# federicomegler/sq-learn

Measured on AMD Instinct MI355X. Metric: q-means fit samples/sec (Lloyd samples*iterations/s, delta-means + tomography noise), higher is better.
Workload: dtype fp32; 1 GPU; model=q-means k=1024 delta=0.5 (10000000 x 256 synthetic), global_batch=10000000, seq_len=256, parallelism=dp1

## Files before the change

### sq_learn_amd/csrc/estep_f32.hip

```cpp
#include "common.h"
#include "band.h"
#include "f16_tile.h"
#include "sq_api.h"

namespace sq {

constexpr int kMaxCand = 16;

#ifndef SQ_SPLIT_ACC_ALL
#define SQ_SPLIT_ACC_ALL 1
#endif
template <int KSD, int TOP = 2>
__global__ void __launch_bounds__(256, 1) estep_f32_kernel(
    const float* __restrict__ X, const _Float16* __restrict__ C, const float* __restrict__ xn,
    int* __restrict__ labels, float* __restrict__ mind, long long* __restrict__ ovf_rows,
    int* __restrict__ ovf_count, double* __restrict__ part, long long n, int k_pad, float alpha,
    float inv_alpha2, float delta_s, RngKey key, long long row_offset, int ovf_cap,
    const long long* __restrict__ rlist, const int* __restrict__ rcount,
    const float* __restrict__ cmax2_p, long long* __restrict__ mrows, int* __restrict__ mcand,
    int* __restrict__ multi_count, unsigned char* __restrict__ xflag, long long mcap) {
  const float Cm = cmax2_p ? sqrtf(*cmax2_p) * (1.0f + 0x1p-16f) : 0.0f;
  constexpr bool SPLIT_ACC = SQ_SPLIT_ACC_ALL || TOP == 3;
  constexpr float kEps3 =
      SPLIT_ACC ? (3.0f * 0x1p-22f + (KSD * 16 + 18.0f) * 0x1p-24f + 2.0f * KSD * 16 * 0x1p-34f) *
// ... 157 lines not shown

  int G = 0;
  stage(0);
  load_raw(blk);
  sync_tile();
  split();
  double my_inertia = 0.0;

  for (; blk < nblk; blk += gridDim.x) {
    const long long row0 = blk * ROWS + wave * 32;
    if constexpr (!PREFETCH) {
      if (blk != (long long)blockIdx.x) {
        load_raw(blk);
        asm volatile("s_waitcnt vmcnt(0)" ::: "memory");
        split();
      }
    }
#pragma unroll
    for (int i = 0; i < 16; ++i) {
      m1[i] = m2[i] = m3[i] = __builtin_inff();
      i1[i] = i2[i] = 0;
      if constexpr (TOP == 3) {
        m4[i] = __builtin_inff();
        i3[i] = 0;
      }
    }
    f32x16 pA0, pA1, pB0, pB1;
    stage(G + 1);
    tile_step(buf(G), pA0, pA1, true, pA0, pA1, 0, false);
    sync_tile();
    int t = 0;
    while (true) {
      if (t + 1 >= n_tiles) {
        if constexpr (PREFETCH) load_raw(blk + gridDim.x);
        tile_step(smem, pB0, pB1, false, pA0, pA1, t, true);
        break;
      }
      stage(G + 2);
      tile_step(buf(G + 1), pB0, pB1, true, pA0, pA1, t, true);
      sync_tile();
      ++t;
      ++G;
      if (t + 1 >= n_tiles) {
        if constexpr (PREFETCH) load_raw(blk + gridDim.x);
        tile_step(smem, pA0, pA1, false, pB0, pB1, t, true);
        break;
      }
      stage(G + 2);
      tile_step(buf(G + 1), pA0, pA1, true, pB0, pB1, t, true);
      sync_tile();
      ++t;
      ++G;
    }
    ++G;

    float R1[16], R2[16];
    int RI[16];
#pragma unroll
    for (int i = 0; i < 16; ++i) { R1[i] = m1[i]; R2[i] = m2[i]; RI[i] = i1[i]; }
#pragma unroll
    for (int o = 16, c = 8; o >= 2; o >>= 1, c >>= 1) {
      const bool hi = (r32 & o) != 0;
#pragma unroll
      for (int j = 0; j < c; ++j) {
        const float ra = R1[j], rb = R1[c + j], sa = R2[j], sb = R2[c + j];
        const int ia = RI[j], ib = RI[c + j];
        const float s1 = hi ? ra : rb, s2 = hi ? sa : sb;
        const int si = hi ? ia : ib;
        float k1 = hi ? rb : ra, k2 = hi ? sb : sa;
        int ki = hi ? ib : ia;
        merge(k1, k2, ki, __shfl_xor(s1, o, 64), __shfl_xor(s2, o, 64), __shfl_xor(si, o, 64));
        R1[j] = k1;
        R2[j] = k2;
        RI[j] = ki;
      }
    }
    float q1 = R1[0], q2 = R2[0];
    int qi = RI[0];
    merge(q1, q2, qi, __shfl_xor(R1[0], 1, 64), __shfl_xor(R2[0], 1, 64), __shfl_xor(RI[0], 1, 64));

    const int irow = r32 >> 1;
    const int rloc = acc_row(irow, half);
    const long long grow_local = row0 + rloc;
    const bool owner = ((r32 & 1) == 0) && grow_local < n;
    const float thr = q1 + delta_s;
    const long long gmap = owner ? map_row(grow_local) : 0;
    const float xnv = owner ? xn[gmap] : 0.0f;
    const float e2 = cmax2_p ? 2.0f * kEps3 * (2.0f * alpha * sqrtf(xnv) * Cm + Cm * Cm) : 0.0f;
    const bool unc = cmax2_p && fabsf(q2 - thr) <= e2;
    const bool band2 = q2 <= thr && !unc;
    if (owner) {
      const float dist = fmaxf(xnv + q1 * inv_alpha2, 0.0f);
      mind[gmap] = dist;
      if (!band2 && !unc) labels[gmap] = qi;
      my_inertia += (double)dist;
    }
    const unsigned long long slow = __ballot(owner && (band2 || unc));
    if (slow) {
      const float urow = band_u(key, row_offset + gmap);
#pragma unroll
      for (int i = 0; i < 16; ++i) {
        const unsigned long long sel = slow & ((1ull << (2 * i)) | (1ull << (32 + 2 * i)));
        if (!sel) continue;
        const int src = 32 * half + 2 * i;
        const bool mine = (slow >> src) & 1ull;
        const float thr_i = __shfl(thr, src, 64);
        const float u_i = __shfl(urow, src, 64);
        const float e2_i = __shfl(e2, src, 64);
        const bool unc_i = __shfl(unc ? 1 : 0, src, 64) != 0;
        const long long g_i = __shfl(gmap, src, 64);
        const int c1 = (mine && m1[i] <= thr_i) ? 1 : 0;
        const int c2 = (mine && m2[i] <= thr_i) ? 1 : 0;
        int c3 = 0;
        bool v3;
        const float lim = thr_i + e2_i;
        bool nr = fabsf(m1[i] - thr_i) <= e2_i || fabsf(m2[i] - thr_i) <= e2_i ||
                  fabsf(m3[i] - thr_i) <= e2_i;
        int cc = (m1[i] <= lim ? 1 : 0) + (m2[i] <= lim ? 1 : 0);
        bool last_in;
        if constexpr (TOP == 3) {
          c3 = (mine && m3[i] <= thr_i) ? 1 : 0;
          v3 = mine && m4[i] <= thr_i;
          nr = nr || fabsf(m4[i] - thr_i) <= e2_i;
          cc += m3[i] <= lim ? 1 : 0;
          last_in = m4[i] <= lim;
        } else {
          v3 = mine && m3[i] <= thr_i;
          last_in = m3[i] <= lim;
        }
        const bool row_unc =
            cmax2_p && mine &&
            (unc_i || ((__ballot(mine && nr) >> (32 * half)) & 0xFFFFFFFFull) != 0ull);
        const int cl = c1 + c2 + c3;
        int incl = cl, cinc = cc;
#pragma unroll
        for (int o = 1; o < 32; o <<= 1) {
          const int v = __shfl_up(incl, o, 32);
          const int w = __shfl_up(cinc, o, 32);
          if (r32 >= o) {
            incl += v;
            cinc += w;
          }
        }
        const int ctot = __shfl(cinc, 32 * half + 31, 64);
        const bool untr = ((__ballot(mine && last_in) >> (32 * half)) & 0xFFFFFFFFull) != 0ull;
        const bool to_multi = row_unc && mrows && !untr && ctot >= 2 && ctot <= kMaxCand;
        if (to_multi) {
          int* mc = mcand + g_i * (kMaxCand + 1);
          const int b0 = 1 + cinc - cc;
          if (cc > 0) mc[b0] = i1[i];
          if (cc > 1) mc[b0 + 1] = i2[i];
          if constexpr (TOP == 3) {
            if (cc > 2) mc[b0 + 2] = i3[i];
          }
        }
        const int total = __shfl(incl, 32 * half + 31, 64);
        const bool ovf = ((__ballot(v3) >> (32 * half)) & 0xFFFFFFFFull) != 0ull;
        const int r = band_rank(u_i, total > 0 ? total : 1);
        const bool hit = cl > 0 && r >= incl - cl && r < incl;
        int myj;
        if constexpr (TOP == 3) {
          const int x1 = i1[i];
          const int x2 = cl >= 2 ? i2[i] : 0x7fffffff, x3 = cl >= 3 ? i3[i] : 0x7fffffff;
          const int s_lo = min(x1, min(x2, x3)), s_hi = max(x1, max(x2, x3));
          const int s_mid = (int)((unsigned)x1 + (unsigned)x2 + (unsigned)x3 - (unsigned)s_lo -
                                  (unsigned)s_hi);
          const int kk = r - (incl - cl);
          myj = kk == 0 ? s_lo : (kk == 1 ? (cl == 2 ? min(max(x1, x2), s_hi) : s_mid) : s_hi);
        } else {
          const int x1 = i1[i], x2 = i2[i];
          const int lo_j = min(x1, x2), hi_j = max(x1, x2);
          myj = cl == 1 ? x1 : (r - (incl - cl) == 0 ? lo_j : hi_j);
        }
        const unsigned long long hb = __ballot(hit) >> (32 * half);
        const int pl = hb ? __ffsll((long long)hb) - 1 : 0;
        const int jsel = __shfl(myj, 32 * half + pl, 64);
        if (mine && r32 == 2 * i) {
          const long long g = gmap;
          bool to_ovf = ovf;
          if (row_unc) {
            to_ovf = false;
            if (to_multi) {
              const long long slot = atomicAdd(multi_count, 1);
              if (slot < mcap) {
                mrows[slot] = g;
                if (xflag) xflag[slot] = 1;
                mcand[g * (kMaxCand + 1)] = ctot;
                labels[g] = -1;
              } else {
                to_ovf = true;
              }
            } else if (ctot == 1 && !untr) {
              labels[g] = qi;
            } else {
              to_ovf = true;
            }
          }
          if (to_ovf) {
            const int slot = atomicAdd(ovf_count, 1);
            if (slot < ovf_cap) ovf_rows[slot] = g;
            labels[g] = -1;
          } else if (!row_unc) {
            labels[g] = jsel;
          }
        }
      }
    }
    if constexpr (PREFETCH) {
      if (blk + gridDim.x < nblk) split();
    }
  }
  my_inertia = wave_sum(my_inertia);
  if (lane == 0) part[(size_t)blockIdx.x * NW + wave] = my_inertia;
  asm volatile("s_waitcnt vmcnt(0)" ::: "memory");
}

constexpr int kGapCand = 4;
struct __align__(16) GapRec {
  float da, err;
  float g[kGapCand];
  unsigned ids[2];
};

constexpr int kX64Waves = 4;

#ifndef SQ_X64_STAMP
#define SQ_X64_STAMP 0
#endif
#if SQ_X64_STAMP
constexpr int kStampWaves = 8192;
constexpr int kStampN = 12;
__device__ unsigned long long g_x64_stamps[kStampWaves * kStampN];
#define SQ_STAMP_NOW() __builtin_amdgcn_s_memtime()
#endif

template <int KSD>
using X64Ring = TileRing<KSD, kX64Waves>;

template <int KSD>
struct X64RowSets {
  static constexpr int value = KSD <= 16 ? 2 : 1;
};
constexpr int kX64Pfd = 2;

template <int KSD, int RS>
__global__ void __launch_bounds__(kX64Waves * 64) estep_x64_kernel(
    const _Float16* __restrict__ Xh, const float* __restrict__ X, const _Float16* __restrict__ C,
    const float* __restrict__ Cm, const float* __restrict__ xn, const float* __restrict__ cmax2_p,
    int* __restrict__ labels, float* __restrict__ mind, long long* __restrict__ dense_rows,
    int* __restrict__ dense_count, long long* __restrict__ mrows, int* __restrict__ mcand,
    int* __restrict__ multi_count, long long n, int k_pad, float alpha, float delta_s,
    RngKey key, long long row_offset, int dense_cap, int qbits, const long long* __restrict__ rlist,
    const int* __restrict__ rcount, float* __restrict__ ub, float* __restrict__ lb,
    int* __restrict__ mflag) {
  constexpr int NW = kX64Waves;
  constexpr int DX = KSD * 16;
  using Ring = X64Ring<KSD>;
  constexpr int KT = Ring::KT, NS = Ring::NS, SK = Ring::SK, RING = Ring::RING;
  constexpr int ROWS = NW * 32 * RS;
  extern __shared__ __attribute__((aligned(16))) unsigned char smem[];
  auto buf = [&](int g) -> unsigned char* { return Ring::buf(smem, g); };
  int* cand_all = reinterpret_cast<int*>(smem + Ring::BYTES);
  int* cnt_all = cand_all + NW * RS * 32 * kMaxCand;

  const int tid = threadIdx.x;
  const int lane = tid & 63;
  const int wave = __builtin_amdgcn_readfirstlane(tid >> 6);
  const int r32 = lane & 31;
  const int half = lane >> 5;
  const int n_tiles = k_pad / kTileN;
  const long long ne = rlist ? min((long long)*rcount, n) : n;
  auto row_at = [&](long long pos) -> long long {
    const long long q = pos < ne ? pos : ne - 1;
    return rlist ? rlist[q] : q;
  };
  const long long nblk = (ne + ROWS - 1) / ROWS;
  long long blk = blockIdx.x;
  if (blk >= nblk) return;
  const uint32_t qmask = (1u << qbits) - 1u;
  const uint32_t keep = ~qmask;
  const float Ch = 2.0f * sqrtf(*cmax2_p) * (1.0f + 0x1p-16f);
  const float pack_rel = ldexpf(1.0f, qbits - 23) + 0x1p-15f;
  const float sub_rel = 0x1p-21f * sqrtf((float)DX);

  auto stage = [&](int U) { Ring::stage(C, smem, U, n_tiles); };

  f16x8 ah[RS][KSD];
  auto load_a = [&](long long b) {
    sq::load_a(ah, half, [&](int st) {
      return Xh + (size_t)row_at(b * ROWS + (wave * RS + st) * 32 + r32) * DX;
    });
  };
  const f16x8 aug = aug_frag(half);
  const int rl_own = acc_row(r32 >> 1, half);
  float xn_cur[RS], xn_nxt[RS];
  auto load_xn = [&](long long b, float (&dst)[RS]) {
#pragma unroll
    for (int st = 0; st < RS; ++st) dst[st] = xn[row_at(b * ROWS + (wave * RS + st) * 32 + rl_own)];
  };

  float m1[RS][16], m2[RS][16], m3[RS][16];
  const int lane_off = f16op::lane_off(half, r32);
  auto ins = [&](int st, int i, float v, uint32_t q) {
    const float p = and_or(v, keep, q);
    const float a1 = m1[st][i], a2 = m2[st][i];
    m3[st][i] = vmed3(a2, p, m3[st][i]);
    m2[st][i] = vmed3(a1, p, a2);
    m1[st][i] = vmin(a1, p);
  };
  typedef f32x16 Acc[RS][2];
  auto sub_step = [&](auto S_, const unsigned char* cur, Acc& acc, const Acc& o, int t_prev,
                      bool do_epi) {
    constexpr int S = decltype(S_)::value;
    constexpr int K0 = S * SK, K1 = (S + 1) * SK < KT ? (S + 1) * SK : KT;
    const uint32_t q0 = (uint32_t)(t_prev * 2), q1 = q0 + 1u;
    const unsigned char* hb = cur + lane_off;
    f16x8 b0[2], b1[2];
    b0[0] = ldb(hb + f16op::frag_off(0, 0));
    b1[0] = ldb(hb + f16op::frag_off(1, 0));
#pragma unroll
    for (int ks = K0; ks < K1; ++ks) {
      const int c = (ks - K0) & 1, nx = c ^ 1;
      if (ks + 1 < K1) {
        b0[nx] = ldb(hb + f16op::frag_off(0, ks + 1 - K0));
        b1[nx] = ldb(hb + f16op::frag_off(1, ks + 1 - K0));
      }
#pragma unroll
      for (int st = 0; st < RS; ++st) {
        const f16x8 A = ks < KSD ? ah[st][ks] : aug;
        acc[st][0] = __builtin_amdgcn_mfma_f32_32x32x16_f16(A, b0[c], acc[st][0], 0, 0, 0);
        acc[st][1] = __builtin_amdgcn_mfma_f32_32x32x16_f16(A, b1[c], acc[st][1], 0, 0, 0);
      }
      if (do_epi) {
#pragma unroll
        for (int e = (ks * 16 * RS) / KT; e < ((ks + 1) * 16 * RS) / KT; ++e) {
          ins(e / 16, e % 16, o[e / 16][0][e % 16], q0);
          ins(e / 16, e % 16, o[e / 16][1][e % 16], q1);
        }
      }
      __builtin_amdgcn_sched_barrier(0);
    }
  };
  auto epi_all = [&](const Acc& o, int t_prev) {
    const uint32_t q0 = (uint32_t)(t_prev * 2), q1 = q0 + 1u;
#pragma unroll
    for (int st = 0; st < RS; ++st)
#pragma unroll
      for (int i = 0; i < 16; ++i) {
        ins(st, i, o[st][0][i], q0);
        ins(st, i, o[st][1][i], q1);
      }
  };
#if SQ_X64_STAMP
  unsigned long long st_sync = 0, st_sync0 = 0, st_post = 0, st_sweep = 0, st_blocks = 0;
  unsigned long long st_stage = 0, st_cand = 0, st_aload = 0, st_rmin = 0, st_cl = 0, st_ub = 0;
  const unsigned long long st_t0 = SQ_STAMP_NOW();
  bool st_first = true;
#endif
  auto sync_tile = [&]() {
#if SQ_X64_STAMP
    const unsigned long long sa = SQ_STAMP_NOW();
#endif
    Ring::sync();
#if SQ_X64_STAMP
    const unsigned long long sw = SQ_STAMP_NOW() - sa;
    st_sync += sw;
    if (st_first) st_sync0 += sw;
    st_first = false;
#endif
  };

  int U = 0;
  auto tile = [&](Acc& acc, const Acc& o, int t_prev, bool do_epi) {
#pragma unroll
    for (int st = 0; st < RS; ++st) acc[st][0] = acc[st][1] = (f32x16){0};
    static_for<NS>([&](auto S_) {
      stage(U + RING - 1);
      sub_step(S_, buf(U), acc, o, t_prev, do_epi);
      sync_tile();
      ++U;
    });
  };

  stage(0);
  stage(1);
  load_a(blk);
  load_xn(blk, xn_cur);
  asm volatile("s_waitcnt vmcnt(0)" ::: "memory");
  __builtin_amdgcn_s_barrier();

  for (; blk < nblk; blk += gridDim.x) {
#pragma unroll
    for (int st = 0; st < RS; ++st)
#pragma unroll
      for (int i = 0; i < 16; ++i) m1[st][i] = m2[st][i] = m3[st][i] = __builtin_inff();
    if constexpr (RS == 1) {
      Acc pA, pB;
      tile(pA, pA, 0, false);
      int t = 0;
      while (true) {
        if (t + 1 >= n_tiles) {
          load_a(blk + gridDim.x);
          load_xn(blk + gridDim.x, xn_nxt);
          epi_all(pA, t);
          break;
        }
        tile(pB, pA, t, true);
        ++t;
        if (t + 1 >= n_tiles) {
          load_a(blk + gridDim.x);
          load_xn(blk + gridDim.x, xn_nxt);
          epi_all(pB, t);
          break;
        }
        tile(pA, pB, t, true);
        ++t;
      }
    } else {
      f32x16 cA[RS], cB[RS];
      constexpr int PFD = kX64Pfd;
      f16x8 bq[PFD + 1];
      static_assert(NS == 1, "row sets need whole tiles per LDS slot");
#if SQ_X64_STAMP
      const unsigned long long sw0 = SQ_STAMP_NOW();
      st_first = true;
      ++st_blocks;
#endif
      for (int t = 0; t < n_tiles; ++t) {
#if SQ_X64_STAMP
        const unsigned long long sg0 = SQ_STAMP_NOW();
#endif
        stage(U + RING - 1);
#if SQ_X64_STAMP
        st_stage += SQ_STAMP_NOW() - sg0;
#endif
        tile_prime<KT>(buf(U), lane_off, bq);
        half_pass<0>(buf(U), lane_off, ah, aug, bq, cA, cB, (uint32_t)(2 * t - 1), t > 0, ins);
        half_pass<1>(buf(U), lane_off, ah, aug, bq, cB, cA, (uint32_t)(2 * t), true, ins);
        sync_tile();
        ++U;
      }
#if SQ_X64_STAMP
      const unsigned long long sl0 = SQ_STAMP_NOW();
#endif
      load_a(blk + gridDim.x);
      load_xn(blk + gridDim.x, xn_nxt);
#if SQ_X64_STAMP
      st_aload += SQ_STAMP_NOW() - sl0;
#endif
      half_drain(cB, (uint32_t)(2 * n_tiles - 1), ins);
#if SQ_X64_STAMP
      st_sweep += SQ_STAMP_NOW() - sw0;
#endif
    }
#if SQ_X64_STAMP
    const unsigned long long sp0 = SQ_STAMP_NOW();
#endif

#pragma nounroll
    for (int st = 0; st < RS; ++st) {
#if SQ_X64_STAMP
    const unsigned long long sc0 = SQ_STAMP_NOW();
#endif
    const long long row0 = blk * ROWS + (wave * RS + st) * 32;
    int* cand = cand_all + (wave * RS + st) * 32 * kMaxCand;
    int* cnt = cnt_all + (wave * RS + st) * 32;
    float ms1[16], ms2[16], ms3[16];
#pragma unroll
    for (int i = 0; i < 16; ++i) {
      ms1[i] = m1[0][i]; ms2[i] = m2[0][i]; ms3[i] = m3[0][i];
#pragma unroll
      for (int o = 1; o < RS; ++o) {
        const float a1 = m1[o][i], a2 = m2[o][i], a3 = m3[o][i];
        ms1[i] = st == o ? a1 : ms1[i];
        ms2[i] = st == o ? a2 : ms2[i];
        ms3[i] = st == o ? a3 : ms3[i];
      }
    }

    auto row_min = [&](float (&R)[16]) -> float {
#pragma unroll
      for (int o = 16, c = 8; o >= 2; o >>= 1, c >>= 1) {
        const bool hi = (r32 & o) != 0;
#pragma unroll
        for (int j = 0; j < c; ++j) {
          const float lo_v = R[j], hi_v = R[c + j];
          const float keepv = hi ? hi_v : lo_v, sendv = hi ? lo_v : hi_v;
          R[j] = vmin(keepv, __shfl_xor(sendv, o, 64));
        }
      }
      return vmin(R[0], __shfl_xor(R[0], 1, 64));
    };
    float R[16];
#pragma unroll
    for (int i = 0; i < 16; ++i) R[i] = ms1[i];
    const float rmin = row_min(R);
    float xn_own = xn_cur[0];
#pragma unroll
    for (int o = 1; o < RS; ++o) xn_own = st == o ? xn_cur[o] : xn_own;
    const float xsv = alpha * sqrtf(xn_own) * (1.0f + 0x1p-16f);
    const float prod = xsv * Ch;
    const float mag = 0.25f * Ch * Ch + prod;
    const float E = 1.0625f * 0x1p-10f * prod + pack_rel * mag + sub_rel * (xsv + Ch);
    const float T_own = __uint_as_float(__float_as_uint(rmin) & keep) + delta_s + 2.0f * E;

#if SQ_X64_STAMP
    const unsigned long long sc1 = SQ_STAMP_NOW();
    st_rmin += sc1 - sc0;
#endif
    float nc[16];
    float Tr[16];
#pragma unroll
    for (int i = 0; i < 16; ++i) Tr[i] = __shfl(T_own, 32 * half + 2 * i, 64);
    int* const sink = cnt_all + NW * RS * 32 + wave * 64 + lane;
#pragma unroll
    for (int i = 0; i < 16; ++i) {
      const float T = Tr[i];
      nc[i] = ms1[i] > T ? ms1[i] : (ms2[i] > T ? ms2[i] : ms3[i]);
      const int rl = acc_row(i, half);
      auto jof = [&](float p) -> int {
        const uint32_t q = __float_as_uint(p) & qmask;
        return (int)((q >> 1) * kTileN + (q & 1u) * 32u) + r32;
      };
      const unsigned long long b1 = __ballot(ms1[i] <= T), b2 = __ballot(ms2[i] <= T);
      const unsigned long long b3 = __ballot(ms3[i] <= T);
      const uint32_t b1l = (uint32_t)b1, b1h = (uint32_t)(b1 >> 32);
      const uint32_t b2l = (uint32_t)b2, b2h = (uint32_t)(b2 >> 32);
      const int c1 = __popc(half ? b1h : b1l), c2 = __popc(half ? b2h : b2l);
      const bool d3 = (half ? (uint32_t)(b3 >> 32) : (uint32_t)b3) != 0u;
      const int s1 = (int)__builtin_amdgcn_mbcnt_hi(b1h, __builtin_amdgcn_mbcnt_lo(b1l, 0u)) -
                     (half ? __popc(b1l) : 0);
      const int s2 = c1 + (int)__builtin_amdgcn_mbcnt_hi(b2h, __builtin_amdgcn_mbcnt_lo(b2l, 0u)) -
                     (half ? __popc(b2l) : 0);
      *((ms1[i] <= T && s1 < kMaxCand) ? cand + rl * kMaxCand + s1 : sink) = jof(ms1[i]);
      *((ms2[i] <= T && s2 < kMaxCand) ? cand + rl * kMaxCand + s2 : sink) = jof(ms2[i]);
      *(r32 == 0 ? cnt + rl : sink) = c1 + c2 + (d3 ? kMaxCand + 1 : 0);
    }
#if SQ_X64_STAMP
    const unsigned long long sc2 = SQ_STAMP_NOW();
    st_cl += sc2 - sc1;
#endif
    float ub_own = 0.f, lb_own = 0.f;
    if (ub) {
      const float ncmin = row_min(nc);
      const float ia2 = 1.0f / (alpha * alpha);
      const float d1 = (__uint_as_float(__float_as_uint(rmin) & keep) + E) * ia2;
      const float d2 = (__uint_as_float(__float_as_uint(ncmin) & keep) - E) * ia2;
      const float marg = 0x1p-20f * (xn_own + fabsf(d1) + fabsf(d2));
      ub_own = sqrtf(fmaxf(xn_own + d1 + marg, 0.f)) * (1.0f + 0x1p-20f);
      lb_own = sqrtf(fmaxf(xn_own + d2 - marg, 0.f)) * (1.0f - 0x1p-20f);
    }
    asm volatile("s_waitcnt lgkmcnt(0)" ::: "memory");
    __builtin_amdgcn_wave_barrier();
#if SQ_X64_STAMP
    st_cand += SQ_STAMP_NOW() - sc0;
    st_ub += SQ_STAMP_NOW() - sc2;
#endif

    const bool valid = row0 + r32 < ne;
    const long long g = row_at(row0 + r32);
    if (ub) {
      const int src = ((r32 & 3) + 4 * ((r32 >> 3) & 3)) * 2 + 32 * ((r32 >> 2) & 1);
      const float u = __shfl(ub_own, src, 64), l = __shfl(lb_own, src, 64);
      if (valid && half == 0) {
        ub[g] = u;
        lb[g] = cnt[r32] <= kMaxCand ? l : 0.0f;
      }
    }
    const int c_r = cnt[r32];
    const bool dense = c_r > kMaxCand;
    const bool multi = valid && !dense && c_r >= 2;
    if (mflag && valid && half == 0 && !multi) mflag[g] = 0;
    if (valid && half == 0) {
      if (dense) {
        const int s = atomicAdd(dense_count, 1);
        if (s < dense_cap) dense_rows[s] = g;
        labels[g] = -1;
      } else if (c_r == 1) {
        labels[g] = cand[r32 * kMaxCand];
        mind[g] = -1.0f;
      }
    }
    const bool mrow = multi && half == 0;
    const unsigned long long mm = __ballot(mrow);
    const int nm = __popcll(mm);
    int mbase = 0;
    if (lane == 0 && nm) mbase = atomicAdd(multi_count, nm);
    mbase = __shfl(mbase, 0, 64);
    if (mrow) {
      const long long slot = (long long)mbase + __popcll(mm & ((1ull << lane) - 1ull));
      if (mflag) mflag[g] = slot < n ? 1 : 0;
      if (slot < n) {
        mrows[slot] = g;
        int* mc = mcand + g * (kMaxCand + 1);
        mc[0] = c_r;
        for (int c = 0; c < c_r; ++c) mc[1 + c] = cand[r32 * kMaxCand + c];
      } else {
        const int s2 = atomicAdd(dense_count, 1);
        if (s2 < dense_cap) dense_rows[s2] = g;
        labels[g] = -1;
      }
    }
    asm volatile("s_waitcnt lgkmcnt(0)" ::: "memory");
    __builtin_amdgcn_wave_barrier();
    }
#pragma unroll
    for (int st = 0; st < RS; ++st) xn_cur[st] = xn_nxt[st];
#if SQ_X64_STAMP
    st_post += SQ_STAMP_NOW() - sp0;
#endif
  }
  asm volatile("s_waitcnt vmcnt(0)" ::: "memory");
#if SQ_X64_STAMP
  const int sidx = blockIdx.x * NW + wave;
  if (lane == 0 && sidx < kStampWaves) {
    unsigned long long* o = g_x64_stamps + (size_t)sidx * kStampN;
    o[0] = SQ_STAMP_NOW() - st_t0; o[1] = st_sweep; o[2] = st_sync; o[3] = st_sync0;
    o[4] = st_post; o[5] = st_blocks; o[6] = st_stage; o[7] = st_cand; o[8] = st_aload;
    o[9] = st_rmin; o[10] = st_cl; o[11] = st_ub;
  }
#endif
}

constexpr int kBfLdsK = 2048;
template <int PER>
__global__ void __launch_bounds__(256) bounds_filter_kernel(
    const int* __restrict__ labels, float* __restrict__ ub, float* __restrict__ lb,
    const double* __restrict__ shift, const double* __restrict__ smax, long long n, double delta,
    long long* __restrict__ rlist, int* __restrict__ rcount, const int* __restrict__ mflag,
    long long* __restrict__ mrows, int* __restrict__ multi_count, const float* __restrict__ cc,
    const int* __restrict__ fidx, int nf, int k, int rec_on, int it_now, int it_lo,
    long long* __restrict__ mrows_b, int* __restrict__ count_b, float* __restrict__ corr,
    int* __restrict__ rec_count) {
  constexpr int kBoundsChunk = PER * 256;
  __shared__ int wsum[4], wsum_b[4];
  __shared__ int lbase[3];
  __shared__ double sf_s[65];
  __shared__ double sh_s[kBfLdsK];
  __shared__ float cm_s[kBfLdsK];
  const bool tab = k <= kBfLdsK;
  const int tid = threadIdx.x, lane = tid & 63, wv = tid >> 6;
  if (tid < nf) sf_s[tid] = shift[fidx[tid]];
  if (tab)
    for (int j = tid; j < k; j += 256) {
      sh_s[j] = shift[j];
      cm_s[j] = nf > 0 ? cc[(size_t)k * nf + j] : 0.0f;
    }
  __syncthreads();
  if (tid == 0) {
    double m = 0.0;
    for (int f = 0; f < nf; ++f) m = fmax(m, sf_s[f]);
    sf_s[nf] = m;
  }
  __syncthreads();
  const double sm = *smax;
  const long long c0 = (long long)blockIdx.x * kBoundsChunk;
  unsigned long long act = 0, rec = 0, recb = 0;
  constexpr int B = PER % 4 == 0 ? 4 : 1;
  for (int p0 = 0; p0 < PER; p0 += B) {
    int lv[B], mfv[B];
    float ubv[B], lbv[B];
    bool inb[B];
#pragma unroll
    for (int q = 0; q < B; ++q) {
      const long long i = c0 + (long long)(p0 + q) * 256 + tid;
      inb[q] = i < n;
      const long long ii = inb[q] ? i : 0;
      lv[q] = inb[q] ? labels[ii] : -1;
      if (corr && inb[q]) corr[ii] = 0.0f;
      ubv[q] = ub[ii];
      lbv[q] = lb[ii];
      mfv[q] = mflag[ii];
    }
    double shv[B];
    float cmv[B];
#pragma unroll
    for (int q = 0; q < B; ++q) {
      const int l = lv[q];
      if (tab) {
        shv[q] = l >= 0 ? sh_s[l] : 1e300;
        cmv[q] = l >= 0 ? cm_s[l] : 0.0f;
      } else {
        shv[q] = l >= 0 ? shift[l] : 1e300;
        cmv[q] = (l >= 0 && nf > 0) ? cc[(size_t)k * nf + l] : 0.0f;
      }
    }
#pragma unroll
    for (int q = 0; q < B; ++q) {
      if (!inb[q]) continue;
      const int p = p0 + q;
      const long long i = c0 + (long long)p * 256 + tid;
      const int l = lv[q];
      const double u = (double)ubv[q] + shv[q];
      auto wbound = [&](double lb0) -> double {
        double w = lb0 - sm;
        if (l >= 0 && nf > 0 && w > 0.0) {
          const double wc = fmin(w, fmax((double)cmv[q] - u, lb0 - sf_s[nf]));
          if (wc > 0.0 && wc * wc - u * u > delta * (1.0 + 1e-9) + 1e-30) {
            w = wc;
          } else {
            const float* cl = cc + (size_t)l * nf;
            if ((nf & 3) == 0) {
              for (int f = 0; f < nf; f += 4) {
                const float4 c4 = *reinterpret_cast<const float4*>(cl + f);
                w = fmin(w, fmax((double)c4.x - u, lb0 - sf_s[f]));
                w = fmin(w, fmax((double)c4.y - u, lb0 - sf_s[f + 1]));
                w = fmin(w, fmax((double)c4.z - u, lb0 - sf_s[f + 2]));
                w = fmin(w, fmax((double)c4.w - u, lb0 - sf_s[f + 3]));
              }
            } else {
              for (int f = 0; f < nf; ++f) w = fmin(w, fmax((double)cl[f] - u, lb0 - sf_s[f]));
            }
          }
        }
        return w;
      };
      const double w = wbound((double)lbv[q]);
      const bool holds = l >= 0 && w > 0.0 && w * w - u * u > delta * (1.0 + 1e-9) + 1e-30;
      if (!holds) {
        act |= 1ull << p;
      } else {
        ub[i] = (float)u * (1.0f + 0x1p-22f);
        lb[i] = (float)w * (1.0f - 0x1p-22f);
        if (mfv[q]) {
          if (rec_on && mfv[q] >= it_lo + 2 && mfv[q] <= it_now + 1) recb |= 1ull << p;
          else rec |= 1ull << p;
        }
      }
    }
  }
  const int mine = __popcll(act) | (__popcll(rec) << 16);
  const int mine_b = __popcll(recb);
  int incl = mine, incl_b = mine_b;
#pragma unroll
  for (int o = 1; o < 64; o <<= 1) {
    const int v = __shfl_up(incl, o, 64);
    const int vb = __shfl_up(incl_b, o, 64);
    if (lane >= o) {
      incl += v;
      incl_b += vb;
    }
  }
  if (lane == 63) {
    wsum[wv] = incl;
    wsum_b[wv] = incl_b;
  }
  __syncthreads();
  int before = 0, total = 0, before_b = 0, total_b = 0;
#pragma unroll
  for (int w2 = 0; w2 < 4; ++w2) {
    before += w2 < wv ? wsum[w2] : 0;
    total += wsum[w2];
    before_b += w2 < wv ? wsum_b[w2] : 0;
    total_b += wsum_b[w2];
  }
  if (tid < 4) {
    const int add = tid == 0 ? (total & 0xffff) : (tid == 2 ? total_b : (total >> 16));
    int* ctr = tid == 0 ? rcount : (tid == 1 ? multi_count : (tid == 2 ? count_b : rec_count));
    const int at = (add && ctr) ? atomicAdd(ctr, add) : 0;
    if (tid < 3) lbase[tid] = at;
  }
  __syncthreads();
  const int ex = before + incl - mine;
  int pos = lbase[0] + (ex & 0xffff);
  while (act) {
    const int p = __ffsll((long long)act) - 1;
    rlist[pos++] = c0 + (long long)p * 256 + tid;
    act &= act - 1;
  }
  int mpos = lbase[1] + (ex >> 16);
  while (rec) {
    const int p = __ffsll((long long)rec) - 1;
    mrows[mpos++] = c0 + (long long)p * 256 + tid;
    rec &= rec - 1;
  }
  int bpos = lbase[2] + before_b + incl_b - mine_b;
  while (recb) {
    const int p = __ffsll((long long)recb) - 1;
    mrows_b[bpos++] = c0 + (long long)p * 256 + tid;
    recb &= recb - 1;
  }
}

struct MultiRec {
  GapRec* rec = nullptr;
  int* mflag = nullptr;
  int it_now = 0, it_lo = 0;
  int ring = 0;
  const _Float16* dsh = nullptr;
  const float* dq = nullptr;
  long long dsh_stride = 0;
  long long* mrows_b = nullptr;
  int* count_b = nullptr;
  int* n_done = nullptr;
  long long* mrows_mv = nullptr;
  int* count_mv = nullptr;
};
struct Ovf2 {
  void* rows = nullptr;
  int* count = nullptr;
};

extern "C" int sq_bounds_filter(const void* labels, void* ub, void* lb, const void* shift,
                                const void* smax, long long n, double delta, void* rlist,
                                void* rcount, const void* mflag, void* mrows, void* multi_count,
                                const void* cc, const void* fidx, int nf, int k, void* stream,
                                void* corr, void* rec_count, int rec_on, int it_now, int it_lo,
                                void* mrows_b, void* count_b) {
  if (rec_on && (it_now < 1 || it_lo < 1 || it_lo > it_now || !mrows_b || !count_b))
    return (int)hipErrorInvalidValue;
  if (n <= 0) return 0;
  if (!mflag || !mrows || !multi_count) return (int)hipErrorInvalidValue;
  if (nf < 0 || nf > 64 || (nf > 0 && (!cc || !fidx || k <= nf))) return (int)hipErrorInvalidValue;
  hipStream_t st = (hipStream_t)stream;
  static long long resident = 0;
  if (resident == 0) {
    int dev = 0, cus = 0, per_cu = 0;
    hipGetDevice(&dev);
    hipDeviceGetAttribute(&cus, hipDeviceAttributeMultiprocessorCount, dev);
    hipOccupancyMaxActiveBlocksPerMultiprocessor(&per_cu, (const void*)bounds_filter_kernel<32>,
                                                 256, 0);
    resident = (long long)(cus > 0 ? cus : 256) * (per_cu > 0 ? per_cu : 4);
  }
  auto pick = [&](int per) { return (n + per * 256LL - 1) / (per * 256LL) <= resident; };
  static const int per_env = [] {
    const char* e = getenv("SQ_BF_PER");
    return e ? atoi(e) : 0;
  }();
  int per = pick(8) ? 8 : pick(16) ? 16 : pick(20) ? 20 : pick(32) ? 32 : 64;
  if (per_env == 4 || per_env == 8 || per_env == 16 || per_env == 20 || per_env == 32 ||
      per_env == 64)
    per = per_env;
  const long long blocks = (n + per * 256LL - 1) / (per * 256LL);
  auto kern = per == 4 ? bounds_filter_kernel<4> : per == 8 ? bounds_filter_kernel<8>
            : per == 16 ? bounds_filter_kernel<16> : per == 20 ? bounds_filter_kernel<20>
            : per == 32 ? bounds_filter_kernel<32> : bounds_filter_kernel<64>;
  hipLaunchKernelGGL(kern, dim3((unsigned)blocks),
                     dim3(256), 0, st, (const int*)labels, (float*)ub, (float*)lb,
                     (const double*)shift, (const double*)smax, n, delta, (long long*)rlist,
// ... 1209 lines not shown
```

### sq_learn_amd/csrc/f16_tile.h

```cpp
#pragma once
#include "common.h"
#include <utility>

namespace sq {

typedef _Float16 f16x8 __attribute__((ext_vector_type(8)));
typedef float f32x16 __attribute__((ext_vector_type(16)));

constexpr int kTileN = 64;

SQ_DEV float vmin(float a, float b) {
  float r;
  asm("v_min_f32 %0, %1, %2" : "=v"(r) : "v"(a), "v"(b));
  return r;
}
SQ_DEV float and_or(float a, uint32_t m, uint32_t q) {
  float r;
  asm("v_and_or_b32 %0, %1, %2, %3" : "=v"(r) : "v"(a), "s"(m), "v"(q));
  return r;
}
SQ_DEV float vmed3(float a, float b, float c) {
  float r;
  asm("v_med3_f32 %0, %1, %2, %3" : "=v"(r) : "v"(a), "v"(b), "v"(c));
  return r;
}

template <typename F, int... I>
SQ_DEV void static_for_impl(F&& f, std::integer_sequence<int, I...>) {
  (f(std::integral_constant<int, I>{}), ...);
}
template <int N, typename F>
SQ_DEV void static_for(F&& f) {
  static_for_impl(f, std::make_integer_sequence<int, N>{});
}

__host__ __device__ constexpr int acc_row(int i, int half) {
  return (i & 3) + 8 * (i >> 2) + 4 * half;
}

namespace f16op {
constexpr int kChunkElems = kTileN * 8;
constexpr int kChunkBytes = kChunkElems * 2;
constexpr int kStepBytes = 2 * kChunkBytes;
constexpr int kColHalfBytes = 32 * 16;
constexpr int kNormElems = 3;

__host__ __device__ constexpr int hi_bytes(int ksd) { return (ksd + 1) * kStepBytes; }
__host__ __device__ constexpr int tile_bytes(int ksd) { return (2 * ksd + 1) * kStepBytes; }

__host__ __device__ constexpr size_t row_base(int d_pad, int j) {
  return (size_t)(j >> 6) * (2 * (d_pad / 8) + 2) * kChunkElems + (size_t)(j & 63) * 8;
}
__host__ __device__ constexpr size_t hi_off(int f) { return (size_t)(f >> 3) * kChunkElems + (f & 7); }
__host__ __device__ constexpr size_t lo_off(int d_pad, int f) {
  return (size_t)(d_pad / 8 + 2 + (f >> 3)) * kChunkElems + (f & 7);
}

__host__ __device__ constexpr int lane_off(int half, int r32) { return (half * 64 + r32) * 16; }
__host__ __device__ constexpr int frag_off(int h, int ks) { return h * kColHalfBytes + ks * kStepBytes; }
}

SQ_DEV f16x8 ldb(const unsigned char* p) { return *reinterpret_cast<const f16x8*>(p); }

template <int KSD, int NW>
struct TileRing {
  static constexpr int RING = 3;
  static constexpr int KT = KSD + 1;
  static constexpr int NS = (KT + 23) / 24;
  static constexpr int SK = (KT + NS - 1) / NS;
  static constexpr int SLOT = SK * f16op::kStepBytes;
  static constexpr int PIECES = SLOT / f16op::kChunkBytes;
  static constexpr int PPW = (PIECES + NW - 1) / NW;
  static constexpr int BYTES = RING * SLOT;

  static SQ_DEV unsigned char* buf(unsigned char* smem, int g) { return smem + (g % RING) * SLOT; }

  static SQ_DEV void stage(const _Float16* C, unsigned char* smem, int U, int n_tiles) {
    const int t = (NS == 1 ? U : U / NS) % n_tiles;
    const int sub = NS == 1 ? 0 : U % NS;
    const int npc = 2 * min(SK, KT - sub * SK);
    const unsigned char* tile = reinterpret_cast<const unsigned char*>(C) +
                                (size_t)t * f16op::tile_bytes(KSD) + (size_t)sub * SLOT;
    unsigned char* dst = buf(smem, U);
#pragma unroll
    for (int i = 0; i < PPW; ++i) {
      const int wave = __builtin_amdgcn_readfirstlane((int)threadIdx.x >> 6);
      const int p = wave + NW * i < npc ? wave + NW * i : npc - 1;
      const int lane = threadIdx.x & 63;
      __builtin_amdgcn_global_load_lds(
          (const __attribute__((address_space(1))) void*)(tile + p * f16op::kChunkBytes + lane * 16),
          (__attribute__((address_space(3))) void*)(dst + p * f16op::kChunkBytes), 16, 0, 0);
    }
  }
  static SQ_DEV void sync() {
    asm volatile("s_waitcnt vmcnt(%0)" ::"n"(PPW) : "memory");
    __builtin_amdgcn_s_barrier();
  }
};

static inline int resident_blocks(const void* kern, int threads, size_t lds) {
  int dev = 0, cus = 0, per_cu = 0;
  (void)hipGetDevice(&dev);
  (void)hipDeviceGetAttribute(&cus, hipDeviceAttributeMultiprocessorCount, dev);
  (void)hipOccupancyMaxActiveBlocksPerMultiprocessor(&per_cu, kern, threads, lds);
  return (cus > 0 ? cus : 256) * (per_cu > 0 ? per_cu : 1);
}

SQ_DEV f16x8 a_frag(const _Float16* row, int half, int ks) {
  return *reinterpret_cast<const f16x8*>(row + half * 8 + ks * 16);
}
template <int RS, int KSD, typename Row>
SQ_DEV void load_a(f16x8 (&ah)[RS][KSD], int half, Row&& row) {
#pragma unroll
  for (int st = 0; st < RS; ++st) {
    const _Float16* xr = row(st);
#pragma unroll
    for (int ks = 0; ks < KSD; ++ks) ah[st][ks] = a_frag(xr, half, ks);
  }
}
SQ_DEV f16x8 aug_frag(int half) {
  f16x8 aug = (f16x8)0;
  if (half == 0) { aug[0] = aug[1] = aug[2] = (_Float16)1.0f; }
  return aug;
}

template <int KT, int NB>
SQ_DEV void tile_prime(const unsigned char* cur, int lane_off, f16x8 (&bq)[NB]) {
#pragma unroll
  for (int j = 0; j < NB - 1; ++j) bq[j] = ldb(cur + lane_off + f16op::frag_off(j / KT, j % KT));
}
template <int H, int KSD, int RS, int NB, typename Epi>
SQ_DEV void half_pass(const unsigned char* cur, int lane_off, const f16x8 (&ah)[RS][KSD],
                      const f16x8& aug, f16x8 (&bq)[NB], f32x16 (&acc)[RS],
                      const f32x16 (&o)[RS], uint32_t qo, bool do_epi, Epi&& epi) {
  constexpr int KT = KSD + 1, PFD = NB - 1;
#pragma unroll
  for (int st = 0; st < RS; ++st) acc[st] = (f32x16){0};
#pragma unroll
  for (int ks = 0; ks < KT; ++ks) {
    const int g = H * KT + ks;
    if (g + PFD < 2 * KT)
      bq[(g + PFD) % NB] = ldb(cur + lane_off + f16op::frag_off((g + PFD) / KT, (g + PFD) % KT));
#pragma unroll
    for (int st = 0; st < RS; ++st)
      acc[st] = __builtin_amdgcn_mfma_f32_32x32x16_f16(ks < KSD ? ah[st][ks] : aug, bq[g % NB],
                                                       acc[st], 0, 0, 0);
    if (do_epi) {
#pragma unroll
      for (int e = (ks * 16 * RS) / KT; e < ((ks + 1) * 16 * RS) / KT; ++e)
        epi(e / 16, e % 16, o[e / 16][e % 16], qo);
    }
    __builtin_amdgcn_sched_barrier(0);
  }
}
template <int RS, typename Epi>
SQ_DEV void half_drain(const f32x16 (&o)[RS], uint32_t qo, Epi&& epi) {
#pragma unroll
  for (int st = 0; st < RS; ++st)
#pragma unroll
    for (int i = 0; i < 16; ++i) epi(st, i, o[st][i], qo);
}

SQ_DEV void tile_from_zero(const unsigned char* tile, int lane_off, const _Float16* row, int half,
                           int ksd, f32x16& c0, f32x16& c1) {
  const f16x8 aug = aug_frag(half);
  c0 = (f32x16){0};
  c1 = (f32x16){0};
  for (int ks = 0; ks < ksd + 1; ++ks) {
    const f16x8 av = ks < ksd ? a_frag(row, half, ks) : aug;
    const f16x8 b0 = ldb(tile + lane_off + f16op::frag_off(0, ks));
    const f16x8 b1 = ldb(tile + lane_off + f16op::frag_off(1, ks));
    c0 = __builtin_amdgcn_mfma_f32_32x32x16_f16(av, b0, c0, 0, 0, 0);
    c1 = __builtin_amdgcn_mfma_f32_32x32x16_f16(av, b1, c1, 0, 0, 0);
  }
}

}
```

Measured before the change: 16.86 billion samples*iter/s.

## Interleave centroid tile staging with MFMA passes and trim candidate-list epilogue

Replaces the bulk per-tile staging call with per-piece global-to-LDS loads spread across the MFMA k-steps of each half pass, tracked by explicit ring-slot and look-ahead tile counters. The epilogue insertion into the top-3 lists is also spread per MFMA and hand-written as inline asm for multi-row-set configs. The goal is to hide load issue and VALU work behind matrix instructions. Separately, the candidate-count code skips the second and third ballot processing when no lane has a qualifying second or third candidate. This adds scheduling complexity, and the inline asm and AGPR constraint hints may increase register pressure.

```diff
diff --git a/sq_learn_amd/csrc/estep_f32.hip b/sq_learn_amd/csrc/estep_f32.hip
--- a/sq_learn_amd/csrc/estep_f32.hip
+++ b/sq_learn_amd/csrc/estep_f32.hip
@@ -483,11 +483,21 @@
   float m1[RS][16], m2[RS][16], m3[RS][16];
   const int lane_off = f16op::lane_off(half, r32);
   auto ins = [&](int st, int i, float v, uint32_t q) {
-    const float p = and_or(v, keep, q);
-    const float a1 = m1[st][i], a2 = m2[st][i];
-    m3[st][i] = vmed3(a2, p, m3[st][i]);
-    m2[st][i] = vmed3(a1, p, a2);
-    m1[st][i] = vmin(a1, p);
+    if constexpr (RS == 1) {
+      const float p = and_or(v, keep, q);
+      const float a1 = m1[st][i], a2 = m2[st][i];
+      m3[st][i] = vmed3(a2, p, m3[st][i]);
+      m2[st][i] = vmed3(a1, p, a2);
+      m1[st][i] = vmin(a1, p);
+    } else {
+      float p;
+      asm("v_and_or_b32 %3, %4, %5, %6\n\t"
+          "v_med3_f32 %2, %1, %3, %2\n\t"
+          "v_med3_f32 %1, %0, %3, %1\n\t"
+          "v_min_f32 %0, %0, %3"
+          : "+v"(m1[st][i]), "+v"(m2[st][i]), "+v"(m3[st][i]), "=&v"(p)
+          : "v"(v), "s"(keep), "v"(q));
+    }
   };
   typedef f32x16 Acc[RS][2];
   auto sub_step = [&](auto S_, const unsigned char* cur, Acc& acc, const Acc& o, int t_prev,
@@ -552,6 +562,8 @@
   };
 
   int U = 0;
+  [[maybe_unused]] int t_ahead = (RING - 1) % n_tiles;
+  [[maybe_unused]] int s_cur = 0;
   auto tile = [&](Acc& acc, const Acc& o, int t_prev, bool do_epi) {
 #pragma unroll
     for (int st = 0; st < RS; ++st) acc[st][0] = acc[st][1] = (f32x16){0};
@@ -611,15 +623,24 @@
 #if SQ_X64_STAMP
         const unsigned long long sg0 = SQ_STAMP_NOW();
 #endif
-        stage(U + RING - 1);
+        unsigned char* const cur = smem + s_cur * Ring::SLOT;
+        unsigned char* const pdst = smem + (s_cur == 0 ? RING - 1 : s_cur - 1) * Ring::SLOT;
+        auto piece = [&](auto G_) {
+          constexpr int g = decltype(G_)::value, I = (g * Ring::PPW) / (2 * KT);
+          if constexpr (g == (I * 2 * KT + Ring::PPW - 1) / Ring::PPW)
+            Ring::template piece<I>(C, t_ahead, pdst);
+        };
 #if SQ_X64_STAMP
         st_stage += SQ_STAMP_NOW() - sg0;
 #endif
-        tile_prime<KT>(buf(U), lane_off, bq);
-        half_pass<0>(buf(U), lane_off, ah, aug, bq, cA, cB, (uint32_t)(2 * t - 1), t > 0, ins);
-        half_pass<1>(buf(U), lane_off, ah, aug, bq, cB, cA, (uint32_t)(2 * t), true, ins);
+        tile_prime<KT>(cur, lane_off, bq);
+        half_pass_paced<0>(cur, lane_off, ah, aug, bq, cA, cB, (uint32_t)(2 * t - 1), t > 0, ins,
+                           piece);
+        half_pass_paced<1>(cur, lane_off, ah, aug, bq, cB, cA, (uint32_t)(2 * t), true, ins, piece);
         sync_tile();
         ++U;
+        s_cur = s_cur + 1 == RING ? 0 : s_cur + 1;
+        t_ahead = t_ahead + 1 == n_tiles ? 0 : t_ahead + 1;
       }
 #if SQ_X64_STAMP
       const unsigned long long sl0 = SQ_STAMP_NOW();
@@ -707,15 +728,20 @@
       const unsigned long long b3 = __ballot(ms3[i] <= T);
       const uint32_t b1l = (uint32_t)b1, b1h = (uint32_t)(b1 >> 32);
       const uint32_t b2l = (uint32_t)b2, b2h = (uint32_t)(b2 >> 32);
-      const int c1 = __popc(half ? b1h : b1l), c2 = __popc(half ? b2h : b2l);
-      const bool d3 = (half ? (uint32_t)(b3 >> 32) : (uint32_t)b3) != 0u;
+      const int c1 = __popc(half ? b1h : b1l);
       const int s1 = (int)__builtin_amdgcn_mbcnt_hi(b1h, __builtin_amdgcn_mbcnt_lo(b1l, 0u)) -
                      (half ? __popc(b1l) : 0);
-      const int s2 = c1 + (int)__builtin_amdgcn_mbcnt_hi(b2h, __builtin_amdgcn_mbcnt_lo(b2l, 0u)) -
-                     (half ? __popc(b2l) : 0);
       *((ms1[i] <= T && s1 < kMaxCand) ? cand + rl * kMaxCand + s1 : sink) = jof(ms1[i]);
-      *((ms2[i] <= T && s2 < kMaxCand) ? cand + rl * kMaxCand + s2 : sink) = jof(ms2[i]);
-      *(r32 == 0 ? cnt + rl : sink) = c1 + c2 + (d3 ? kMaxCand + 1 : 0);
+      int c23 = 0;
+      if ((b2 | b3) != 0ull) {
+        const int c2 = __popc(half ? b2h : b2l);
+        const bool d3 = (half ? (uint32_t)(b3 >> 32) : (uint32_t)b3) != 0u;
+        const int s2 = c1 + (int)__builtin_amdgcn_mbcnt_hi(b2h, __builtin_amdgcn_mbcnt_lo(b2l, 0u)) -
+                       (half ? __popc(b2l) : 0);
+        *((ms2[i] <= T && s2 < kMaxCand) ? cand + rl * kMaxCand + s2 : sink) = jof(ms2[i]);
+        c23 = c2 + (d3 ? kMaxCand + 1 : 0);
+      }
+      *(r32 == 0 ? cnt + rl : sink) = c1 + c23;
     }
 #if SQ_X64_STAMP
     const unsigned long long sc2 = SQ_STAMP_NOW();
diff --git a/sq_learn_amd/csrc/f16_tile.h b/sq_learn_amd/csrc/f16_tile.h
--- a/sq_learn_amd/csrc/f16_tile.h
+++ b/sq_learn_amd/csrc/f16_tile.h
@@ -92,6 +92,20 @@
           (__attribute__((address_space(3))) void*)(dst + p * f16op::kChunkBytes), 16, 0, 0);
     }
   }
+  template <int I>
+  static SQ_DEV void piece(const _Float16* C, int t, unsigned char* slot) {
+    static_assert(NS == 1 && I < PPW, "pieces of a whole-tile slot");
+    const int wave = __builtin_amdgcn_readfirstlane((int)threadIdx.x >> 6);
+    const unsigned lane = threadIdx.x & 63;
+    unsigned p = wave + NW * I;
+    if constexpr (NW * I + NW - 1 >= PIECES) p = min(p, (unsigned)(PIECES - 1));
+    const unsigned off = p * f16op::kChunkBytes;
+    __builtin_amdgcn_global_load_lds(
+        (const __attribute__((address_space(1))) void*)(
+            reinterpret_cast<const unsigned char*>(C) +
+            (size_t)((unsigned)t * (unsigned)f16op::tile_bytes(KSD) + off + lane * 16u)),
+        (__attribute__((address_space(3))) void*)(slot + off), 16, 0, 0);
+  }
   static SQ_DEV void sync() {
     asm volatile("s_waitcnt vmcnt(%0)" ::"n"(PPW) : "memory");
     __builtin_amdgcn_s_barrier();
@@ -152,6 +166,36 @@
     }
     __builtin_amdgcn_sched_barrier(0);
   }
+}
+template <int H, int KSD, int RS, int NB, typename Epi, typename Fill>
+SQ_DEV void half_pass_paced(const unsigned char* cur, int lane_off, const f16x8 (&ah)[RS][KSD],
+                            const f16x8& aug, f16x8 (&bq)[NB], f32x16 (&acc)[RS],
+                            const f32x16 (&o)[RS], uint32_t qo, bool do_epi, Epi&& epi,
+                            Fill&& fill) {
+  constexpr int KT = KSD + 1, PFD = NB - 1, NM = KT * RS, NE = 16 * RS;
+#pragma unroll
+  for (int st = 0; st < RS; ++st) acc[st] = (f32x16){0};
+  static_for<KT>([&](auto KS_) {
+    constexpr int ks = decltype(KS_)::value, g = H * KT + ks;
+    if constexpr (g + PFD < 2 * KT)
+      bq[(g + PFD) % NB] = ldb(cur + lane_off + f16op::frag_off((g + PFD) / KT, (g + PFD) % KT));
+    fill(std::integral_constant<int, g>{});
+#pragma unroll
+    for (int st = 0; st < RS; ++st) {
+      acc[st] = __builtin_amdgcn_mfma_f32_32x32x16_f16(ks < KSD ? ah[st][ks] : aug, bq[g % NB],
+                                                       acc[st], 0, 0, 0);
+      if (do_epi) {
+        const int m = ks * RS + st;
+#pragma unroll
+        for (int e = (m * NE) / NM; e < ((m + 1) * NE) / NM; ++e) {
+          float v = o[e / 16][e % 16];
+          asm("" : "+a"(v));
+          epi(e / 16, e % 16, v, qo);
+        }
+      }
+      __builtin_amdgcn_sched_barrier(0);
+    }
+  });
 }
 template <int RS, typename Epi>
 SQ_DEV void half_drain(const f32x16 (&o)[RS], uint32_t qo, Epi&& epi) {
```

Measured after the change: 16.85 billion samples*iter/s. Within noise of the previous version (-0.0%).
